# zhoujoey/ORB-SLAM3-Mac

Measured on AMD Instinct MI355X. Metric: ORB extract+match frames/sec, higher is better.
Workload: dtype u8; 1 GPU; vga: synthetic 640x480 batch=1024 per GPU, 8-level pyramid, 1000 feats/frame, ORB extract + Hamming 2-NN match (Frame.cc:1146) + SearchForInitialization (ORBmatcher.cc:710) vs successor frame; pipelines=1, matchers=side by side (two contexts), frames_total=1024

## Files before the change

include/orbhip.h:

```cpp
#ifndef ORBHIP_H
#define ORBHIP_H
#include <stddef.h>
#include <stdint.h>
#ifdef __cplusplus
extern "C" {
#endif

#define ORBHIP_OK 0
#define ORBHIP_E_BADARG (-1)
#define ORBHIP_E_NODEVICE (-2)
#define ORBHIP_E_HIP (-3)
#define ORBHIP_E_CAPACITY (-4)
#define ORBHIP_E_ABORTED (-5)
#define ORBHIP_E_NOTSPD (-6)
#define ORBHIP_E_EMPTY (-7)

typedef struct {
    float x, y, size, angle, response;
    int32_t octave, class_id;
} orbhip_keypoint;

typedef struct orbhip_ctx orbhip_ctx;
typedef struct orbhip_extractor orbhip_extractor;

// ... 3 lines not shown
int orbhip_ctx_create(int device, void *stream, orbhip_ctx **out);
void orbhip_ctx_destroy(orbhip_ctx *ctx);
int orbhip_ctx_synchronize(orbhip_ctx *ctx);
int orbhip_ctx_wait_for(orbhip_ctx *ctx, orbhip_ctx *other);
int orbhip_ctx_check_status(orbhip_ctx *ctx);
void *orbhip_ctx_stream(orbhip_ctx *ctx);

int orbhip_extractor_create(orbhip_ctx *ctx, int nfeatures, float scale_factor, int nlevels,
                            int ini_th_fast, int min_th_fast, orbhip_extractor **out);
void orbhip_extractor_destroy(orbhip_extractor *ext);

int orbhip_extractor_levels(const orbhip_extractor *ext);
int orbhip_extractor_table(const orbhip_extractor *ext, int which, float *out);
int orbhip_extractor_features_per_level(const orbhip_extractor *ext, int *out);
int orbhip_extractor_umax(const orbhip_extractor *ext, int *out16);

int orbhip_extractor_reserve(orbhip_extractor *ext, int width, int height, int max_batch);
int orbhip_extractor_max_keypoints(const orbhip_extractor *ext);

int orbhip_extract_batch_device(orbhip_extractor *ext, const uint8_t *d_images, int width,
                                int height, size_t row_stride, size_t frame_stride, int batch,
                                int lap0, int lap1);
int orbhip_extractor_results(orbhip_extractor *ext, orbhip_keypoint **d_kp, uint8_t **d_desc,
                             int32_t **d_count, int32_t **d_mono_index);
int orbhip_extract_batch_host(orbhip_extractor *ext, const uint8_t *h_images, int width, int height,
                              size_t row_stride, size_t frame_stride, int batch, int lap0, int lap1,
                              orbhip_keypoint *kp_out, uint8_t *desc_out, int cap,
                              int32_t *count_out, int32_t *mono_out);
int orbhip_extract_batch_host_view(orbhip_extractor *ext, const uint8_t *h_images, int width, int height, size_t row_stride,
                                   size_t frame_stride, int batch, int lap0, int lap1, const orbhip_keypoint **kp_view,
                                   const uint8_t **desc_view, int *row_capacity, const int32_t **count_view, const int32_t **mono_view);
int orbhip_extractor_blur_kernel(const orbhip_extractor *ext, int batch);

int orbhip_extractor_resize_band_rows(const orbhip_extractor *ext, int level);

int orbhip_extractor_last_frame(orbhip_extractor *ext, int frame, const orbhip_keypoint **d_kp, const uint8_t **d_desc,
                                const orbhip_keypoint **h_kp_view, const uint8_t **h_desc_view, int32_t *count, unsigned long long *generation);

int orbhip_extractor_level_dims(const orbhip_extractor *ext, int level, int *w, int *h);
int orbhip_extractor_get_pyramid_level(orbhip_extractor *ext, int frame, int level, int padded,
                                       uint8_t *h_out, size_t out_stride);
int orbhip_extractor_get_pyramid_padded(orbhip_extractor *ext, int frame, uint8_t *const *levels_out, const size_t *strides);
int orbhip_extractor_get_blurred_level(orbhip_extractor *ext, int frame, int level,
                                       uint8_t *h_out, size_t out_stride);
int orbhip_extractor_get_fast_candidates(orbhip_extractor *ext, int frame, int level,
                                         int32_t *xs, int32_t *ys, int32_t *scores, int cap,
                                         int32_t *n_out);
// ... 575 lines not shown
```

orb-slam3-mac_amd/csrc/orb_internal.h:

```cpp
#pragma once
#include <hip/hip_runtime.h>
#include <stdint.h>
#include "../../include/orbhip.h"

#define ORB_MAX_LEVELS 16
#define ORB_EDGE 19
#define ORB_MINB 16
#define ORB_HALF_PATCH 15
#define ORB_RS_STEPS 24

struct OrbLevel {
    uint8_t *img;
    uint8_t *blur;
    size_t img_frame_stride;
    size_t blur_frame_stride;
    int w, h, img_pitch, blur_pitch;
    int ncols, nrows, wcell, hcell;
    int cell_base;
    int cell_cap;
    int quota;
    int key_base, key_cap;
    int kp_base, kp_cap;
    int n_ini;
    float hx;
    float scale;
    float size;
    const int16_t *xofs; const int16_t *xalpha; const int16_t *yofs; const int16_t *ybeta;
    const uint32_t *xchunk; const uint32_t *ytab;
    int resize_mode;
    int rs_rows;
};
// ... 25 lines not shown
    float *lvl_angle;
    uint8_t *lvl_desc;
    int32_t *lvl_count;
    int32_t *lvl_ncand;
    int32_t *status;
    orbhip_keypoint *out_kp;
    uint8_t *out_desc;
    int32_t *out_count;
    int32_t *out_mono;
    int umax[ORB_HALF_PATCH + 1];
    int gauss_q8[7];
    const uint4 *bm_th;
    const uint4 *bm_tv;
    int bm_cols[ORB_MAX_LEVELS + 1];
    int bm_init;
};

struct FcLevel {
    const uint8_t *img; size_t frame_stride; int img_pitch;
    int max_bx, max_by;
    int ncols, nrows, wcell, hcell, cell_base, cell_cap;
    int tpr, rpt;
    int rpc, rpr, run_base;
};
struct FastParams {
    FcLevel lv[ORB_MAX_LEVELS];
    int nlevels, batch, ini_th, min_th, cells_per_frame;
    int n_cus;
    int chunk;
    int lvl_lo, lvl_hi;
    uint32_t *cell_count, *cell_list; size_t cell_list_frame_stride; int32_t *status;
    int rows, srows, qcap, wave_dw, small_cells;
    uint32_t div_magic[34];
    int runs_per_frame, run_rows, run_q0, run_dw, use_runs;
};

#define ORB_PACK_KEY(x, y, s) ((uint32_t)(x) | ((uint32_t)(y) << 12) | ((uint32_t)(s) << 24))
#define ORB_KEY_X(k) ((int)((k) & 0xFFFu))
#define ORB_KEY_Y(k) ((int)(((k) >> 12) & 0xFFFu))
#define ORB_KEY_S(k) ((int)((k) >> 24))

__device__ __forceinline__ int hamming256(const uint4 &a0, const uint4 &a1, const uint4 &b0, const uint4 &b1)
{
    return __popc(a0.x ^ b0.x) + __popc(a0.y ^ b0.y) + __popc(a0.z ^ b0.z) + __popc(a0.w ^ b0.w) +
           __popc(a1.x ^ b1.x) + __popc(a1.y ^ b1.y) + __popc(a1.z ^ b1.z) + __popc(a1.w ^ b1.w);
}

struct StereoLevel {
    const uint8_t *imgL, *imgR;
    size_t fsL, fsR;
    int pitchL, pitchR, wR, pad_;
// ... 33 lines not shown
```

orb-slam3-mac_amd/csrc/orb_kernels.hip:

```cpp
#include "orb_internal.h"
#include "wave_dpp.h"
#include <mutex>
#include <vector>
#include <cstdio>
#include <cstdlib>

#define WAVE 64

__device__ __forceinline__ int wave_incl_scan(int v) { return wave_scan_add_dpp(v); }

__device__ __forceinline__ int block_excl_scan256(int v, int *wsum, int *total)
{
    const int lane = threadIdx.x & (WAVE - 1), wid = threadIdx.x >> 6;
    int inc = wave_incl_scan(v);
    if (lane == WAVE - 1) wsum[wid] = inc;
    __syncthreads();
    int base = 0;
#pragma unroll
    for (int w = 0; w < 4; w++) {
        int s = wsum[w];
        if (w < wid) base += s;
    }
    *total = wsum[0] + wsum[1] + wsum[2] + wsum[3];
    __syncthreads();
// ... 1609 lines not shown
    const uint32_t khi = (uint32_t)P.gauss_q8[4] | ((uint32_t)P.gauss_q8[5] << 8) | ((uint32_t)P.gauss_q8[6] << 16);
    const uint32_t k0 = P.gauss_q8[0], k1 = P.gauss_q8[1], k2 = P.gauss_q8[2], k3 = P.gauss_q8[3];
    const uint32_t k01 = k0 | (k1 << 16), k23 = k2 | (k3 << 16), k21 = k2 | (k1 << 16);
    if (idx < nint * nb) {
        const int band = idx / nint, c = 1 + idx - band * nint;
        blr_band<false>(src, dst, L.img_pitch, L.blur_pitch, w, h, 4 * c, band * BLR_R, klo, khi, k01, k23, k21, k0);
    } else {
        const int e = idx - nint * nb, band = e / nedge, ce = e - band * nedge;
        const int c = ce == 0 ? 0 : nint + ce;
        blr_band<true>(src, dst, L.img_pitch, L.blur_pitch, w, h, 4 * c, band * BLR_R, klo, khi, k01, k23, k21, k0);
    }
}

typedef int v4i __attribute__((ext_vector_type(4)));
__device__ __forceinline__ v4i bm_as_v4i(uint4 v) { v4i r; r[0] = (int)v.x; r[1] = (int)v.y; r[2] = (int)v.z; r[3] = (int)v.w; return r; }
__global__ __launch_bounds__(256) void k_blur_mfma(OrbParams P, int frame0, int nframes)
{
    const int per_frame = P.bm_cols[P.nlevels];
    const unsigned wid = xcd_logical_id(blockIdx.x, gridDim.x) * 4 + (threadIdx.x >> 6);
    const int lane = threadIdx.x & 63, m = lane & 15, g = lane >> 4;
    const int fr = (int)(wid / (unsigned)per_frame), rem = (int)(wid - (unsigned)fr * (unsigned)per_frame);
    if (fr >= nframes) return;
    int level = 0;
    for (int l = 1; l < P.nlevels; l++) if (rem >= P.bm_cols[l]) level = l;
    const OrbLevel &L = P.lv[level];
    const int w = L.w, h = L.h, spitch = L.img_pitch, dpitch = L.blur_pitch;
    const int tx = rem - P.bm_cols[level], X0 = 32 * tx;
    const uint8_t *src = L.img + (size_t)(frame0 + fr) * L.img_frame_stride;
    uint8_t *dst = L.blur + (size_t)(frame0 + fr) * L.blur_frame_stride;
    int cx = X0 - 16 + 16 * g;
    cx = cx < 0 ? 0 : cx;
    if (cx + 16 > w) cx = w - 16;
    const uint4 *th = P.bm_th + ((size_t)(P.bm_cols[level] + tx) * 2) * 64 + lane;
    const v4i B0 = bm_as_v4i(th[0]), B1 = bm_as_v4i(th[64]);
    v4i TV[4];
#pragma unroll
    for (int b = 0; b < 4; b++) TV[b] = bm_as_v4i(P.bm_tv[b * 64 + lane]);
    const int init = P.bm_init;
    v4i c_init = {init, init, init, init}, c_init_lo = {init + 32768, init + 32768, init + 32768, init + 32768};
    asm volatile("" : "+v"(c_init), "+v"(c_init_lo));
    const int nty = (h + 57) / 58;
    auto load_window = [&](int Y0, u32x4_unaligned (&raw)[4]) {
// ... 30 lines not shown
                const uint32_t pab = __builtin_amdgcn_perm((uint32_t)C1[cb][t][1], (uint32_t)C1[cb][t][0], 0x05040100u);
                const uint32_t pcd = __builtin_amdgcn_perm((uint32_t)C1[cb][t][3], (uint32_t)C1[cb][t][2], 0x05040100u);
                Alo[t] = (int)(__builtin_amdgcn_perm(pcd, pab, 0x06040200u) ^ 0x80808080u);
                Ahi[t] = (int)(__builtin_amdgcn_perm(pcd, pab, 0x07050301u) ^ 0x80808080u);
            }
            const int col = X0 + 16 * cb + 4 * g;
#pragma unroll
            for (int b = 0; b < 4; b++) {
                const v4i Chi = __builtin_amdgcn_mfma_i32_16x16x64_i8(Ahi, TV[b], c_init, 0, 0, 0);
                const v4i Clo = __builtin_amdgcn_mfma_i32_16x16x64_i8(Alo, TV[b], c_init_lo, 0, 0, 0);
                uint32_t v[4];
#pragma unroll
                for (int r = 0; r < 4; r++) v[r] = min(((uint32_t)Chi[r] << 8) + (uint32_t)Clo[r], 0x00FFFFFFu);
                const uint32_t p01 = __builtin_amdgcn_perm(v[1], v[0], 0x0c0c0602u), p23 = __builtin_amdgcn_perm(v[3], v[2], 0x0c0c0602u);
                const int row = Y0 + 16 * b + m;
                if (16 * b + m < 58 && row < h && col < w) *reinterpret_cast<uint32_t *>(dst + (uint32_t)(__umul24((uint32_t)row, (uint32_t)dpitch) + (uint32_t)col)) = p01 | (p23 << 16);
            }
        }
    }
}

void orb_launch_blur(const OrbParams &P, hipStream_t s, int wgs_per_cu, int frame0, int nframes)
{
    if (P.bm_cols[P.nlevels] > 0 && P.batch >= P.bm_min_batch) {
        if (nframes < 0) nframes = P.batch - frame0;
        const long waves = (long)P.bm_cols[P.nlevels] * nframes;
        if (nframes > 0) hipLaunchKernelGGL(k_blur_mfma, dim3((unsigned)((waves + 3) / 4)), dim3(256), 0, s, P, frame0, nframes);
        return;
    }
    if (P.br_blocks[P.nlevels] > 0 && P.batch >= P.rows_min_batch) {
        if (nframes < 0) nframes = P.batch - frame0;
        if (nframes > 0) hipLaunchKernelGGL(k_blur_rows, dim3((unsigned)P.br_blocks[P.nlevels] * (unsigned)nframes), dim3(256), 0, s, P, frame0);
        return;
    }
    if (frame0 > 0) return;
    const long total = (long)P.bs_tiles[P.nlevels] * P.batch;
    long nblocks = (long)(P.n_cus > 0 ? P.n_cus : 256) * wgs_per_cu;
    if (nblocks > total) nblocks = total;
    hipLaunchKernelGGL(k_blur, dim3((unsigned)nblocks), dim3(256), 0, s, P);
}

__constant__ int8_t c_pattern[1024] = {
// ... 178 lines not shown
            const uint32_t c0 = __float_as_uint(__fadd_rn(__fsub_rn(__fmul_rn(pk.x, a), __fmul_rn(pk.y, b)), MAGIC));
            const uint32_t r1 = __float_as_uint(__fadd_rn(__fadd_rn(__fmul_rn(pk.z, b), __fmul_rn(pk.w, a)), MAGIC));
            const uint32_t c1 = __float_as_uint(__fadd_rn(__fsub_rn(__fmul_rn(pk.z, a), __fmul_rn(pk.w, b)), MAGIC));
            const uint32_t i0 = (r0 << 5) + (r0 << 4) + c0 + offk, i1 = (r1 << 5) + (r1 << 4) + c1 + offk;
            const uint32_t t0 = bp[i0], t1 = bp[i1];
            bits = __builtin_amdgcn_alignbit(bits, t0 - t1, 31);
        }
        if (valid) {
            uint8_t *desc = P.lvl_desc + ((size_t)frame * P.kps_per_frame + slot) * 32;
            reinterpret_cast<uint16_t *>(desc)[l16] = (uint16_t)bits;
            if (l16 == 0) P.lvl_angle[(size_t)frame * P.kps_per_frame + slot] = angle;
        }
    }
}

void orb_launch_orient_desc(const OrbParams &P, hipStream_t s)
{
    const long groups_x = (long)((P.batch + 7) / 8) * ((P.kps_per_frame + 3) >> 2);
    long blocks_x = (groups_x + (OD_THREADS / 64) - 1) / (OD_THREADS / 64);
    if (blocks_x > 4096) blocks_x = 4096;
    const long blocks = 8 * blocks_x;
    hipLaunchKernelGGL(k_orient_desc, dim3((unsigned)blocks), dim3(OD_THREADS), 0, s, P);
}

__global__ __launch_bounds__(256) void k_assemble(OrbParams P)
{
    __shared__ int wsum[8];
    __shared__ int s_cnt[ORB_MAX_LEVELS + 1];
    const int tid = threadIdx.x, frame = blockIdx.x;
    if (tid == 0) {
        int n = 0;
        for (int l = 0; l < P.nlevels; l++) { s_cnt[l] = n; n += P.lvl_count[frame * P.nlevels + l]; }
        s_cnt[P.nlevels] = n;
    }
    __syncthreads();
    const int n = s_cnt[P.nlevels];
    orbhip_keypoint *okp = P.out_kp + (size_t)frame * P.max_kp;
// ... 42 lines not shown
```

orb-slam3-mac_amd/csrc/orbhip_api.hip:

```cpp
#include "orb_internal.h"
#include "ctx_internal.h"
#include <cmath>
#include <cfloat>
#include <cstdio>
#include <cstdlib>
#include <cstring>
#include <string>
#include <vector>
#include <mutex>
#include <set>
#include <utility>

static thread_local std::string g_last_error;
extern "C" const char *orbhip_last_error(void) { return g_last_error.c_str(); }
extern "C" const char *orbhip_version(void) { return "orbhip 0.1 (gfx950)"; }

#define HIP_TRY(expr)                                                                   \
    do {                                                                                \
        hipError_t _e = (expr);                                                         \
        if (_e != hipSuccess) {                                                         \
            g_last_error = std::string(#expr) + ": " + hipGetErrorString(_e);           \
            return ORBHIP_E_HIP;                                                        \
        }                                                                               \
    } while (0)
// ... 334 lines not shown
    for (int d = 0; d < dn; d++) {
        float f = (float)((d + 0.5) * scale - 0.5);
        int s = (int)floorf(f);
        f -= s;
        if (horizontal) {
            if (s < 0) { f = 0; s = 0; }
            if (s >= sn - 1) { f = 0; s = sn - 1; }
        }
        int c0 = cv_round_f((1.f - f) * 2048), c1 = cv_round_f(f * 2048);
        ofs[d] = (int16_t)std::min(std::max(s, -32768), 32767);
        coef[2 * d] = (int16_t)std::min(std::max(c0, -32768), 32767);
        coef[2 * d + 1] = (int16_t)std::min(std::max(c1, -32768), 32767);
    }
}

extern "C" int orbhip_extractor_reserve(orbhip_extractor *e, int width, int height, int max_batch)
{
    if (!e || width <= 0 || height <= 0 || max_batch <= 0) return ORBHIP_E_BADARG;
    if (e->width == width && e->height == height && e->max_batch >= max_batch) return ORBHIP_OK;
    if (width > 4096 + 2 * ORB_MINB || height > 4096 + 2 * ORB_MINB) { g_last_error = "image larger than 12-bit key packing"; return ORBHIP_E_BADARG; }
    HIP_TRY(hipSetDevice(e->ctx->device));
    HIP_TRY(hipStreamSynchronize(e->ctx->stream));
    ext_free_all(e);
    OrbParams &P = e->P;
    memset(&P, 0, sizeof(P));
    P.nlevels = e->nlevels; P.ini_th = e->ini_th; P.min_th = e->min_th;
    memcpy(P.umax, e->umax, sizeof(P.umax));
    memcpy(P.gauss_q8, e->gauss_q8, sizeof(P.gauss_q8));
    int cells = 0, keys = 0, kps = 0, max_cell_cap = 0;
    for (int l = 0; l < e->nlevels; l++) {
// ... 75 lines not shown
        bool ok = !getenv("ORBHIP_BLUR_TILES");
        P.br_blocks[0] = 0;
        for (int l = 0; l < e->nlevels; l++) {
            const int w = P.lv[l].w, h = P.lv[l].h;
            if (h < BLR_R + 4 || w < 16) ok = false;
            P.br_blocks[l + 1] = P.br_blocks[l] + (((w + 3) / 4) * ((h + BLR_R - 1) / BLR_R) + 255) / 256;
        }
        if (!ok) P.br_blocks[e->nlevels] = 0;
    }
    P.cell_list_frame_stride = (size_t)cells * max_cell_cap;
    int rc;
    const size_t B = (size_t)max_batch;
    for (int l = 0; l < e->nlevels; l++) {
        OrbLevel &L = P.lv[l];
        L.img_pitch = align_up(L.w, 64); L.blur_pitch = L.img_pitch;
        L.img_frame_stride = (size_t)L.img_pitch * L.h; L.blur_frame_stride = L.img_frame_stride;
        if ((rc = dev_alloc(e, &L.img, B * L.img_frame_stride + 64))) return rc;
        if ((rc = dev_alloc(e, &L.blur, B * L.blur_frame_stride + 64))) return rc;
        if (l > 0) {
            std::vector<int16_t> xo, xa, yo, yb;
            resize_tables(P.lv[l - 1].w, L.w, true, xo, xa);
            resize_tables(P.lv[l - 1].h, L.h, false, yo, yb);
            int16_t *dxo, *dxa, *dyo, *dyb;
            if ((rc = dev_alloc(e, &dxo, xo.size()))) return rc;
            if ((rc = dev_alloc(e, &dxa, xa.size()))) return rc;
            if ((rc = dev_alloc(e, &dyo, yo.size()))) return rc;
            if ((rc = dev_alloc(e, &dyb, yb.size()))) return rc;
            HIP_TRY(hipMemcpy(dxo, xo.data(), xo.size() * 2, hipMemcpyHostToDevice));
            HIP_TRY(hipMemcpy(dxa, xa.data(), xa.size() * 2, hipMemcpyHostToDevice));
            HIP_TRY(hipMemcpy(dyo, yo.data(), yo.size() * 2, hipMemcpyHostToDevice));
            HIP_TRY(hipMemcpy(dyb, yb.data(), yb.size() * 2, hipMemcpyHostToDevice));
// ... 92 lines not shown
                            for (int g = 0; g < 4 && gp < 0; g++) if (col >= cxs[g] && col < cxs[g] + 16) gp = g;
                            if (gp < 0) { ok = false; break; }
                            int8_t &c = th[((((size_t)(P.bm_cols[l] + tx) * 2 + cb) * 64) + (size_t)(n + 16 * gp)) * 16 + (col - cxs[gp])];
                            c = (int8_t)(c + e->gauss_q8[i + 3]);
                        }
                    }
            }
        }
        for (int b = 0; b < 4; b++)
            for (int lane = 0; lane < 64; lane++)
                for (int j = 0; j < 16; j++) {
                    const int n = lane & 15, g = lane >> 4, krow = 16 * (j >> 2) + 4 * g + (j & 3), d = krow - (16 * b + n);
                    tv[((size_t)b * 64 + lane) * 16 + j] = (int8_t)((d >= 0 && d <= 6) ? e->gauss_q8[d] : 0);
                }
        P.bm_th = nullptr; P.bm_tv = nullptr; P.bm_init = 128 * S;
        if (ok) {
            uint4 *dth, *dtv;
            if ((rc = dev_alloc(e, &dth, th.size() / 16))) return rc;
            if ((rc = dev_alloc(e, &dtv, tv.size() / 16))) return rc;
            HIP_TRY(hipMemcpy(dth, th.data(), th.size(), hipMemcpyHostToDevice));
            HIP_TRY(hipMemcpy(dtv, tv.data(), tv.size(), hipMemcpyHostToDevice));
            P.bm_th = dth; P.bm_tv = dtv;
        } else P.bm_cols[e->nlevels] = 0;
    }
    if ((rc = dev_alloc(e, &P.cell_count, B * cells))) return rc;
    if ((rc = dev_alloc(e, &P.cell_list, B * P.cell_list_frame_stride))) return rc;
    if ((rc = dev_alloc(e, &P.keys, B * keys))) return rc;
    if ((rc = dev_alloc(e, &P.node_of, B * keys))) return rc;
    if ((rc = dev_alloc(e, &P.lvl_kp, B * kps))) return rc;
    if ((rc = dev_alloc(e, &P.lvl_perm, B * kps))) return rc;
    if ((rc = dev_alloc(e, &P.lvl_angle, B * kps))) return rc;
    if ((rc = dev_alloc(e, &P.lvl_desc, B * kps * 32))) return rc;
    if ((rc = dev_alloc(e, &P.lvl_count, B * e->nlevels))) return rc;
    if ((rc = dev_alloc(e, &P.lvl_ncand, B * e->nlevels))) return rc;
    if ((rc = dev_alloc(e, &P.status, 1))) return rc;
    {
        auto up = [](size_t v) { return (v + 255) & ~(size_t)255; };
        e->ob_kp = up(8 * B); e->ob_desc = e->ob_kp + up(sizeof(orbhip_keypoint) * B * P.max_kp);
        e->outblob_bytes = e->ob_desc + up((size_t)32 * B * P.max_kp);
// ... 151 lines not shown
    memcpy(depth_out, h + 2 * (size_t)max_n, 4 * (size_t)n_left);
    memcpy(x3d_out, h + 3 * (size_t)max_n, 12 * (size_t)n_left);
    if (n_matches_out) *n_matches_out = h[6 * (size_t)max_n];
    return ORBHIP_OK;
}

extern "C" int orbhip_extractor_blur_kernel(const orbhip_extractor *e, int batch)
{
    if (!e || !e->max_batch) return -1;
    const OrbParams &P = e->P;
    if (P.bm_cols[e->nlevels] > 0 && batch >= P.bm_min_batch) return 2;
    if (P.br_blocks[e->nlevels] > 0 && batch >= P.rows_min_batch) return 1;
    return 0;
}

extern "C" int orbhip_extractor_resize_band_rows(const orbhip_extractor *e, int level)
{
    if (!e || !e->max_batch || level < 1 || level >= e->nlevels) return -1;
    return e->P.lv[level].xchunk ? e->P.lv[level].rs_rows : 0;
}

extern "C" int orbhip_extractor_set_profiling(orbhip_extractor *e, int enable)
{
    if (!e) return ORBHIP_E_BADARG;
    if (enable && !e->ev_created) {
        for (auto &slot : e->ev) for (auto &ev : slot) HIP_TRY(hipEventCreate(&ev));
        e->ev_created = true;
    }
    e->profiling = enable != 0;
    e->ev_calls = 0;
// ... 12 lines not shown
            float ms = 0.f;
            HIP_TRY(hipEventElapsedTime(&ms, e->ev[slot][i], e->ev[slot][i + 1]));
            ms_out[i] += ms / n;
        }
    }
    e->ev_calls = 0;
    return ORBHIP_OK;
}

static int tune_int(const char *name, int dflt) { const char *v = getenv(name); return v ? atoi(v) : dflt; }

static int run_pipeline(orbhip_extractor *e, int batch, int lap0, int lap1)
{
    OrbParams &P = e->P;
    P.batch = batch; P.lap0 = lap0; P.lap1 = lap1; P.n_cus = e->ctx->n_cus;
    hipStream_t s = e->ctx->stream;
    const bool prof = e->profiling;
    const int slot = e->ev_calls % ORBHIP_PROF_SLOTS;
#define STAGE_MARK(i) do { if (prof) HIP_TRY(hipEventRecord(e->ev[slot][i], s)); } while (0)
    const bool fork = e->overlap && !prof && batch >= ORB_OVERLAP_MIN_BATCH;
    if (fork && !e->aux_ok) {
        HIP_TRY(hipStreamCreateWithFlags(&e->aux, hipStreamNonBlocking));
        HIP_TRY(hipEventCreateWithFlags(&e->ev_fork, hipEventDisableTiming));
        HIP_TRY(hipEventCreateWithFlags(&e->ev_join, hipEventDisableTiming));
        HIP_TRY(hipEventCreateWithFlags(&e->ev_pyr, hipEventDisableTiming));
        e->aux_ok = true;
    }
    FastParams &F = e->F;
    for (int l = 0; l < e->nlevels; l++) { F.lv[l].img = P.lv[l].img; F.lv[l].frame_stride = P.lv[l].img_frame_stride; F.lv[l].img_pitch = P.lv[l].img_pitch; }
    F.batch = batch; F.n_cus = e->ctx->n_cus; F.cell_count = P.cell_count; F.cell_list = P.cell_list; F.cell_list_frame_stride = P.cell_list_frame_stride; F.status = P.status;
// ... 280 lines not shown
        }
        for (int y = 0; y < ORB_EDGE; y++) {
            memcpy(base + (size_t)y * st, base + (size_t)(ORB_EDGE + reflect101_host(y - ORB_EDGE, L.h)) * st, (size_t)L.w + 2 * ORB_EDGE);
            memcpy(base + (size_t)(L.h + ORB_EDGE + y) * st, base + (size_t)(ORB_EDGE + reflect101_host(L.h + y, L.h)) * st, (size_t)L.w + 2 * ORB_EDGE);
        }
    }
    return ORBHIP_OK;
}

extern "C" int orbhip_extractor_get_blurred_level(orbhip_extractor *e, int frame, int level, uint8_t *h_out, size_t out_stride)
{
    if (!e || !h_out || level < 0 || level >= e->nlevels || frame < 0 || frame >= e->last_batch) return ORBHIP_E_BADARG;
    const OrbLevel &L = e->P.lv[level];
    HIP_TRY(hipSetDevice(e->ctx->device));
    HIP_TRY(hipStreamSynchronize(e->ctx->stream));
    HIP_TRY(hipMemcpy2D(h_out, out_stride, L.blur + (size_t)frame * L.blur_frame_stride, L.blur_pitch, L.w, L.h, hipMemcpyDeviceToHost));
    return ORBHIP_OK;
}

extern "C" int orbhip_extractor_get_fast_candidates(orbhip_extractor *e, int frame, int level, int32_t *xs, int32_t *ys,
                                                    int32_t *scores, int cap, int32_t *n_out)
{
    if (!e || level < 0 || level >= e->nlevels || frame < 0 || frame >= e->last_batch || !n_out) return ORBHIP_E_BADARG;
    const OrbParams &P = e->P;
    const OrbLevel &L = P.lv[level];
    HIP_TRY(hipSetDevice(e->ctx->device));
    HIP_TRY(hipStreamSynchronize(e->ctx->stream));
    int32_t n = 0;
    HIP_TRY(hipMemcpy(&n, P.lvl_ncand + frame * P.nlevels + level, sizeof(n), hipMemcpyDeviceToHost));
    *n_out = n;
// ... 86 lines not shown
```

orb-slam3-mac_amd/python/orbhip.py:

```python
import ctypes as C
import os
import numpy as np

try:
    import torch
except Exception:
    torch = None

_HERE = os.path.dirname(os.path.abspath(__file__))
LIB_DIR = os.path.join(os.path.dirname(_HERE), "lib")
LIB_PATH = os.path.join(LIB_DIR, "liborbhip.so")
SYNTH_PATH = os.path.join(LIB_DIR, "libsynth.so")

if not os.path.exists(LIB_PATH):
    raise ImportError(
        "liborbhip.so not built: run `python -c 'import __graft_entry__ as g; g.build()'` "
        "(there is no CPU fallback for the HIP path)")

lib = C.CDLL(LIB_PATH)

OK, E_BADARG, E_NODEVICE, E_HIP, E_CAPACITY, E_ABORTED, E_NOTSPD, E_EMPTY = 0, -1, -2, -3, -4, -5, -6, -7
STAGES = ["pyramid", "fast_cells", "blur", "octree", "desc", "assemble"]

KP_DTYPE = np.dtype([("x", "<f4"), ("y", "<f4"), ("size", "<f4"), ("angle", "<f4"),
# ... 2 lines not shown

vp, ci, cf, cd, sz = C.c_void_p, C.c_int, C.c_float, C.c_double, C.c_size_t
lib.orbhip_version.restype = C.c_char_p
lib.orbhip_last_error.restype = C.c_char_p
lib.orbhip_ctx_create.argtypes = [ci, vp, C.POINTER(vp)]
lib.orbhip_ctx_destroy.argtypes = [vp]
lib.orbhip_ctx_synchronize.argtypes = [vp]
lib.orbhip_ctx_stream.argtypes = [vp]
lib.orbhip_ctx_stream.restype = vp
lib.orbhip_extractor_create.argtypes = [vp, ci, cf, ci, ci, ci, C.POINTER(vp)]
lib.orbhip_extractor_destroy.argtypes = [vp]
lib.orbhip_extractor_levels.argtypes = [vp]
lib.orbhip_extractor_table.argtypes = [vp, ci, vp]
lib.orbhip_extractor_features_per_level.argtypes = [vp, vp]
lib.orbhip_extractor_umax.argtypes = [vp, vp]
lib.orbhip_extractor_reserve.argtypes = [vp, ci, ci, ci]
lib.orbhip_extractor_max_keypoints.argtypes = [vp]
lib.orbhip_extract_batch_device.argtypes = [vp, vp, ci, ci, sz, sz, ci, ci, ci]
lib.orbhip_extractor_results.argtypes = [vp, C.POINTER(vp), C.POINTER(vp), C.POINTER(vp), C.POINTER(vp)]
lib.orbhip_extract_batch_host.argtypes = [vp, vp, ci, ci, sz, sz, ci, ci, ci, vp, vp, ci, vp, vp]
lib.orbhip_extractor_level_dims.argtypes = [vp, ci, C.POINTER(ci), C.POINTER(ci)]
lib.orbhip_extractor_get_pyramid_level.argtypes = [vp, ci, ci, ci, vp, sz]
lib.orbhip_extractor_get_blurred_level.argtypes = [vp, ci, ci, vp, sz]
lib.orbhip_extractor_get_pyramid_padded.argtypes = [vp, ci, vp, vp]
lib.orbhip_extractor_get_fast_candidates.argtypes = [vp, ci, ci, vp, vp, vp, ci, C.POINTER(C.c_int32)]
lib.orbhip_extractor_get_level_keypoints.argtypes = [vp, ci, ci, vp, ci, C.POINTER(C.c_int32)]
lib.orbhip_extractor_set_profiling.argtypes = [vp, ci]
lib.orbhip_extractor_set_graph_mode.argtypes = [vp, ci]
lib.orbhip_extractor_stage_ms.argtypes = [vp, vp]
lib.orbhip_descriptor_distance.argtypes = [vp, vp]
lib.orbhip_match_bf2nn_device.argtypes = [vp, vp, vp, sz, vp, vp, sz, ci, ci, cd, vp, vp, vp]
lib.orbhip_search_for_initialization_device.argtypes = [vp, vp, vp, vp, vp, vp, vp, ci, ci, sz, cf, cf, cf, cf, ci, cf, ci,
                                                        vp, vp, vp]
lib.orbhip_ctx_check_status.argtypes = [vp]
lib.orbhip_ctx_wait_for.argtypes = [vp, vp]
lib.orbhip_extractor_blur_kernel.argtypes = [vp, ci]
lib.orbhip_extractor_blur_kernel.restype = ci
lib.orbhip_extractor_resize_band_rows.argtypes = [vp, ci]
lib.orbhip_extractor_resize_band_rows.restype = ci
if hasattr(lib, "orbhip_debug_octree"):
    lib.orbhip_debug_octree.argtypes = [vp, ci, ci, vp, vp, vp, vp, ci, vp, ci, vp, vp]
lib.orbhip_prev_matched_init_device.argtypes = [vp, vp, sz, ci, ci, vp]
lib.orbhip_search_by_projection_device.argtypes = [vp, vp, vp, vp, ci, vp, vp, vp, vp, ci, sz, ci, cf, cf, cf, cf, ci, ci, vp, vp]
lib.orbhip_search_local_map_device.argtypes = [vp, vp, vp, vp, ci, vp, vp, vp, vp, ci, sz, ci, cf, cf, cf, cf, ci, cf, vp, vp]


class OrbHipError(RuntimeError):
    def __init__(self, code, where):
        self.code = code
        super().__init__("%s failed: %d (%s)" % (where, code, lib.orbhip_last_error().decode()))


# ... 15 lines not shown
        _chk(lib.orbhip_ctx_check_status(self.h), "orbhip_ctx_check_status")

    def wait_for(self, other):
        _chk(lib.orbhip_ctx_wait_for(self.h, other.h), "orbhip_ctx_wait_for")

    @property
    def stream(self):
        return lib.orbhip_ctx_stream(self.h)

    def close(self):
        if self.h:
            lib.orbhip_ctx_destroy(self.h)
            self.h = None


class Extractor:

    def __init__(self, ctx, nfeatures=1000, scale_factor=1.2, nlevels=8, ini_th=20, min_th=7):
        h = vp()
        _chk(lib.orbhip_extractor_create(ctx.h, nfeatures, scale_factor, nlevels, ini_th, min_th, C.byref(h)),
             "orbhip_extractor_create")
        self.h, self.ctx, self.nlevels = h, ctx, nlevels

    def close(self):
        if self.h:
            lib.orbhip_extractor_destroy(self.h)
            self.h = None

    def table(self, which):
        out = np.zeros(self.nlevels, np.float32)
# ... 7 lines not shown

    def umax(self):
        out = np.zeros(16, np.int32)
        _chk(lib.orbhip_extractor_umax(self.h, out.ctypes.data), "umax")
        return out

    def reserve(self, w, h, batch):
        _chk(lib.orbhip_extractor_reserve(self.h, w, h, batch), "orbhip_extractor_reserve")

    @property
    def max_keypoints(self):
        return lib.orbhip_extractor_max_keypoints(self.h)

    def blur_kernel(self, batch):
        return ("k_blur", "k_blur_rows", "k_blur_mfma")[lib.orbhip_extractor_blur_kernel(self.h, int(batch))]

    def resize_band_rows(self, level):
        return lib.orbhip_extractor_resize_band_rows(self.h, int(level))

    def debug_octree(self, level, lists, form):
        offs = np.zeros(len(lists) + 1, np.int32)
        offs[1:] = np.cumsum([len(l[0]) for l in lists])
        xs, ys, ss = (np.ascontiguousarray(np.concatenate([np.asarray(l[k], np.int32) for l in lists] + [np.zeros(1, np.int32)])) for k in range(3))
        cap = int(max(len(l[0]) for l in lists)) + 16
        keys = np.zeros((len(lists), cap), np.uint32)
        counts, redo = np.zeros(len(lists), np.int32), np.zeros(len(lists), np.int32)
        _chk(lib.orbhip_debug_octree(self.h, int(level), len(lists), offs.ctypes.data, xs.ctypes.data, ys.ctypes.data, ss.ctypes.data,
                                     {"iterative": 0, "table": 1}[form], keys.ctypes.data, cap, counts.ctypes.data, redo.ctypes.data),
             "orbhip_debug_octree")
        kept = [np.stack([k & 0xFFF, (k >> 12) & 0xFFF, k >> 24], 1).astype(np.int32) for k in (keys[f, :counts[f]] for f in range(len(lists)))]
# ... 1114 lines not shown
```

Baseline: 339,300 frames/s.

## Store blurred pyramid in 16x8 tiles and read only pattern-covered rows

The MFMA blur kernel can now write the blurred image in a tiled layout of 16x8-byte tiles. A new orient/descriptor kernel reads the 37x37 blurred neighbourhood from those tiles as 16-byte loads, skipping chunks outside the circular reach of the BRIEF pattern through precomputed per-row half-widths. The goal is fewer wasted and scattered global loads in descriptor computation. In exchange it adds a second layout path, a larger blur buffer, and a host-side untiling step when reading blurred levels back for debugging.

```diff
diff --git a/include/orbhip.h b/include/orbhip.h
--- a/include/orbhip.h
+++ b/include/orbhip.h
@@ -41,6 +41,7 @@
 int orbhip_extractor_table(const orbhip_extractor *ext, int which, float *out);
 int orbhip_extractor_features_per_level(const orbhip_extractor *ext, int *out);
 int orbhip_extractor_umax(const orbhip_extractor *ext, int *out16);
+int orbhip_blur_half_widths(int *out19);
 
 int orbhip_extractor_reserve(orbhip_extractor *ext, int width, int height, int max_batch);
 int orbhip_extractor_max_keypoints(const orbhip_extractor *ext);
@@ -58,6 +59,7 @@
                                    size_t frame_stride, int batch, int lap0, int lap1, const orbhip_keypoint **kp_view,
                                    const uint8_t **desc_view, int *row_capacity, const int32_t **count_view, const int32_t **mono_view);
 int orbhip_extractor_blur_kernel(const orbhip_extractor *ext, int batch);
+int orbhip_extractor_blur_tiled(const orbhip_extractor *ext, int batch);
 
 int orbhip_extractor_resize_band_rows(const orbhip_extractor *ext, int level);
 
diff --git a/orb-slam3-mac_amd/csrc/orb_internal.h b/orb-slam3-mac_amd/csrc/orb_internal.h
--- a/orb-slam3-mac_amd/csrc/orb_internal.h
+++ b/orb-slam3-mac_amd/csrc/orb_internal.h
@@ -15,6 +15,7 @@
     size_t img_frame_stride;
     size_t blur_frame_stride;
     int w, h, img_pitch, blur_pitch;
+    int blur_tiles_x;
     int ncols, nrows, wcell, hcell;
     int cell_base;
     int cell_cap;
@@ -70,6 +71,9 @@
     const uint4 *bm_tv;
     int bm_cols[ORB_MAX_LEVELS + 1];
     int bm_init;
+    int blur_tiled_ok;
+    int blur_tiled;
+    int blur_hw[ORB_EDGE];
 };
 
 struct FcLevel {
@@ -91,6 +95,7 @@
     int runs_per_frame, run_rows, run_q0, run_dw, use_runs;
 };
 
+#define ORB_BLUR_TILE_OFF(x, y, tiles_x) ((((uint32_t)((y) >> 3) * (uint32_t)(tiles_x) + (uint32_t)((x) >> 4)) << 7) + (uint32_t)(((y) & 7) << 4) + (uint32_t)((x) & 15))
 #define ORB_PACK_KEY(x, y, s) ((uint32_t)(x) | ((uint32_t)(y) << 12) | ((uint32_t)(s) << 24))
 #define ORB_KEY_X(k) ((int)((k) & 0xFFFu))
 #define ORB_KEY_Y(k) ((int)(((k) >> 12) & 0xFFFu))
diff --git a/orb-slam3-mac_amd/csrc/orb_kernels.hip b/orb-slam3-mac_amd/csrc/orb_kernels.hip
--- a/orb-slam3-mac_amd/csrc/orb_kernels.hip
+++ b/orb-slam3-mac_amd/csrc/orb_kernels.hip
@@ -1647,6 +1647,7 @@
 
 typedef int v4i __attribute__((ext_vector_type(4)));
 __device__ __forceinline__ v4i bm_as_v4i(uint4 v) { v4i r; r[0] = (int)v.x; r[1] = (int)v.y; r[2] = (int)v.z; r[3] = (int)v.w; return r; }
+template <bool TILED>
 __global__ __launch_bounds__(256) void k_blur_mfma(OrbParams P, int frame0, int nframes)
 {
     const int per_frame = P.bm_cols[P.nlevels];
@@ -1658,7 +1659,7 @@
     for (int l = 1; l < P.nlevels; l++) if (rem >= P.bm_cols[l]) level = l;
     const OrbLevel &L = P.lv[level];
     const int w = L.w, h = L.h, spitch = L.img_pitch, dpitch = L.blur_pitch;
-    const int tx = rem - P.bm_cols[level], X0 = 32 * tx;
+    const int tx = rem - P.bm_cols[level], X0 = 32 * tx, tiles_x = L.blur_tiles_x;
     const uint8_t *src = L.img + (size_t)(frame0 + fr) * L.img_frame_stride;
     uint8_t *dst = L.blur + (size_t)(frame0 + fr) * L.blur_frame_stride;
     int cx = X0 - 16 + 16 * g;
@@ -1719,6 +1720,9 @@
                 for (int r = 0; r < 4; r++) v[r] = min(((uint32_t)Chi[r] << 8) + (uint32_t)Clo[r], 0x00FFFFFFu);
                 const uint32_t p01 = __builtin_amdgcn_perm(v[1], v[0], 0x0c0c0602u), p23 = __builtin_amdgcn_perm(v[3], v[2], 0x0c0c0602u);
                 const int row = Y0 + 16 * b + m;
+                if (TILED) {
+                    if (16 * b + m < 58 && row < h && col < w) *reinterpret_cast<uint32_t *>(dst + ORB_BLUR_TILE_OFF(col, row, tiles_x)) = p01 | (p23 << 16);
+                } else
                 if (16 * b + m < 58 && row < h && col < w) *reinterpret_cast<uint32_t *>(dst + (uint32_t)(__umul24((uint32_t)row, (uint32_t)dpitch) + (uint32_t)col)) = p01 | (p23 << 16);
             }
         }
@@ -1730,7 +1734,8 @@
     if (P.bm_cols[P.nlevels] > 0 && P.batch >= P.bm_min_batch) {
         if (nframes < 0) nframes = P.batch - frame0;
         const long waves = (long)P.bm_cols[P.nlevels] * nframes;
-        if (nframes > 0) hipLaunchKernelGGL(k_blur_mfma, dim3((unsigned)((waves + 3) / 4)), dim3(256), 0, s, P, frame0, nframes);
+        if (nframes > 0 && P.blur_tiled) hipLaunchKernelGGL(k_blur_mfma<true>, dim3((unsigned)((waves + 3) / 4)), dim3(256), 0, s, P, frame0, nframes);
+        else if (nframes > 0) hipLaunchKernelGGL(k_blur_mfma<false>, dim3((unsigned)((waves + 3) / 4)), dim3(256), 0, s, P, frame0, nframes);
         return;
     }
     if (P.br_blocks[P.nlevels] > 0 && P.batch >= P.rows_min_batch) {
@@ -1939,13 +1944,162 @@
     }
 }
 
+#define OD_TP 64
+#define OD_TROWS 40
+#define OD_KP_LDS_T ((OD_TROWS * OD_TP) / 4)
+__global__ __launch_bounds__(OD_THREADS) void k_orient_desc_tiled(OrbParams P)
+{
+    __shared__ __attribute__((aligned(16))) uint32_t lds_all[OD_THREADS / 16][OD_KP_LDS_T];
+    __shared__ float4 pat_t[16 * 16];
+    __shared__ int od_hw[48];
+    __shared__ uint32_t od_msk[16 * 8];
+    const int tid = threadIdx.x, lane = tid & 63, l16 = lane & 15, sub = lane >> 4;
+    for (int e = tid; e < 256; e += OD_THREADS) {
+        const int l = e & 15, t = e >> 4;
+        const int8_t *pp = &c_pattern[4 * (16 * l + t)];
+        pat_t[t * 16 + l] = make_float4((float)pp[0], (float)pp[1], (float)pp[2], (float)pp[3]);
+    }
+    if (tid < 16 * 8) {
+        const int d = P.umax[tid >> 3], j = tid & 7;
+        uint32_t m = 0;
+        for (int k = 0; k < 4; k++) { const int u = -ORB_HALF_PATCH + 4 * j + k; if (u >= -d && u <= d) m |= 0xFFu << (8 * k); }
+        od_msk[tid] = m;
+    }
+    if (tid < 48) { const int r = tid - 3, d = r < 18 ? 18 - r : r - 18; od_hw[tid] = (r >= 0 && r <= 36) ? P.blur_hw[d] : -64; }
+    int uhw[6];
+#pragma unroll
+    for (int k = 0; k < 6; k++) { const int i = l16 + 16 * k, r = (i * 43) >> 7, d = r < 15 ? 15 - r : r - 15; uhw[k] = i < 31 * 3 ? P.umax[d] : -64; }
+    __syncthreads();
+    const int xcd = blockIdx.x & 7, nblk_x = gridDim.x >> 3;
+    const long wave_x = (long)(blockIdx.x >> 3) * (OD_THREADS / 64) + (tid >> 6), nwaves_x = (long)nblk_x * (OD_THREADS / 64);
+    const int gpf = (P.kps_per_frame + 3) >> 2;
+    const int nframes_x = (P.batch - xcd + 7) >> 3;
+    uint32_t *up32 = lds_all[(tid >> 4)], *bp32 = up32;
+    const uint8_t *bp = reinterpret_cast<const uint8_t *>(bp32);
+    const float factor_pi = (float)(3.1415926535897932384626433832795 / 180.f);
+    const long ngroups = (long)nframes_x * gpf;
+    for (long q = wave_x; q < ngroups; q += nwaves_x) {
+        const int fk = __builtin_amdgcn_readfirstlane((int)(q / gpf));
+        const int frame = xcd + 8 * fk;
+        const int slot0 = __builtin_amdgcn_readfirstlane(4 * (int)(q - (long)fk * gpf));
+        int lvl = 0;
+        for (int l = 1; l < P.nlevels; l++) if (slot0 >= P.lv[l].kp_base) lvl = l;
+        lvl = __builtin_amdgcn_readfirstlane(lvl);
+        const OrbLevel &L = P.lv[lvl];
+        const int slot_w = slot0 + sub;
+        const int nk = P.lvl_count[frame * P.nlevels + lvl];
+        const bool valid = (slot_w - L.kp_base) < nk;
+        const int slot = (valid && P.batch >= ORB_PERM_MIN_BATCH) ? L.kp_base + (int)P.lvl_perm[(size_t)frame * P.kps_per_frame + slot_w] : slot_w;
+        if (slot0 - L.kp_base >= nk) continue;
+        int x = 19, y = 19;
+        if (valid) {
+            const uint32_t key = P.lvl_kp[(size_t)frame * P.kps_per_frame + slot];
+            x = ORB_KEY_X(key) + ORB_MINB; y = ORB_KEY_Y(key) + ORB_MINB;
+        }
+        const int uxs = (x - 15) & ~3, uoff = (x - 15) - uxs;
+        const int tc0 = (x - 18) >> 4, boff = (x - 18) & 15, yoff = (y - 18) & 3;
+        __builtin_amdgcn_fence(__ATOMIC_RELEASE, "wavefront");
+        uint4 br[10];
+        uint32_t bmask = 0, umask = 0;
+#pragma unroll
+        for (int k = 0; k < 10; k++) br[k] = make_uint4(0, 0, 0, 0);
+        int bhw[10];
+#pragma unroll
+        for (int k = 0; k < 10; k++) bhw[k] = od_hw[4 * k + (l16 & 3) - yoff + 3];
+        if (valid) {
+            const uint8_t *uimg = L.img + (size_t)frame * L.img_frame_stride, *bimg = L.blur + (size_t)frame * L.blur_frame_stride;
+            const int upitch = L.img_pitch & 0xFFFF, tiles_x = L.blur_tiles_x & 0xFFFF;
+            const uint32_t urow = (uint32_t)(((y - 15) & 0xFFFF) * upitch);
+            const int blo = 16 * (l16 >> 2) - 18 - boff;
+            uint4 ur[6];
+#pragma unroll
+            for (int k = 0; k < 6; k++) {
+                const int i = l16 + 16 * k, r = (i * 43) >> 7, c3 = i - r * 3;
+                const int ulo = 16 * c3 - 15 - uoff;
+                const bool on = ulo <= uhw[k] && ulo + 15 >= -uhw[k];
+                ur[k] = on ? od_load16(uimg, urow + (uint32_t)(r * upitch), uxs + 16 * c3) : make_uint4(0, 0, 0, 0);
+                umask |= on ? 1u << k : 0u;
+            }
+#pragma unroll
+            for (int k = 0; k < 10; k++) {
+                const int gy = y - 18 - yoff + (l16 & 3) + 4 * k;
+                if (blo <= bhw[k] && blo + 15 >= -bhw[k]) {
+                    br[k] = *reinterpret_cast<const uint4 *>(bimg + ((((uint32_t)(gy >> 3) * (uint32_t)tiles_x + (uint32_t)(tc0 + (l16 >> 2))) << 7) + (uint32_t)((gy & 7) << 4)));
+                    bmask |= 1u << k;
+                }
+            }
+#pragma unroll
+            for (int k = 0; k < 6; k++) {
+                const int i = l16 + 16 * k, r = (i * 43) >> 7, c3 = i - r * 3;
+                if (umask & (1u << k)) *reinterpret_cast<uint4 *>(&up32[r * (OD_UP / 4) + 4 * c3]) = ur[k];
+            }
+        }
+        __builtin_amdgcn_fence(__ATOMIC_RELEASE, "wavefront");
+        __builtin_amdgcn_s_waitcnt(0xc07f);
+        __builtin_amdgcn_wave_barrier();
+        __builtin_amdgcn_fence(__ATOMIC_ACQUIRE, "wavefront");
+        int m10, m01 = 0;
+        {
+            const int j = l16 & 7, par = l16 >> 3;
+            const uint32_t wts = 0x04030201u + 0x04040404u * (uint32_t)j;
+            uint32_t accP = 0, accS = 0;
+#pragma unroll 4
+            for (int i = 0; i < 16; i++) {
+                const int v = -ORB_HALF_PATCH + 2 * i + par, vc = min(v, ORB_HALF_PATCH);
+                const uint32_t *rq = up32 + (vc + ORB_HALF_PATCH) * (OD_UP / 4) + j;
+                uint32_t wv = __builtin_amdgcn_alignbyte(rq[1], rq[0], (uint32_t)uoff) & od_msk[(vc < 0 ? -vc : vc) * 8 + j];
+                if (v > ORB_HALF_PATCH) wv = 0;
+                const uint32_t sr = __builtin_amdgcn_udot4(wv, 0x01010101u, 0u, false);
+                accP = __builtin_amdgcn_udot4(wv, wts, accP, false);
+                accS += sr;
+                m01 += v * (int)sr;
+            }
+            m10 = (int)accP - 16 * (int)accS;
+        }
+        __builtin_amdgcn_fence(__ATOMIC_RELEASE, "wavefront");
+        __builtin_amdgcn_wave_barrier();
+#pragma unroll
+        for (int k = 0; k < 10; k++)
+            if (bmask & (1u << k)) *reinterpret_cast<uint4 *>(&bp32[((l16 & 3) + 4 * k) * (OD_TP / 4) + 4 * (l16 >> 2)]) = br[k];
+        m10 = row16_allreduce_add_dpp(m10); m01 = row16_allreduce_add_dpp(m01);
+        const float angle = fast_atan2_deg((float)m01, (float)m10);
+        double sd, cd;
+        sincos_det((double)__fmul_rn(angle, factor_pi), &sd, &cd);
+        const float a = (float)cd, b = (float)sd;
+        __builtin_amdgcn_fence(__ATOMIC_RELEASE, "wavefront");
+        __builtin_amdgcn_s_waitcnt(0xc07f);
+        __builtin_amdgcn_wave_barrier();
+        __builtin_amdgcn_fence(__ATOMIC_ACQUIRE, "wavefront");
+        const float MAGIC = 12582912.0f;
+        const uint32_t offk = (uint32_t)((18 + yoff) * OD_TP + boff + 18) - 65u * 0x4B400000u;
+        uint32_t bits = 0;
+#pragma unroll 4
+        for (int t = 15; t >= 0; t--) {
+            const float4 pk = pat_t[t * 16 + l16];
+            const uint32_t r0 = __float_as_uint(__fadd_rn(__fadd_rn(__fmul_rn(pk.x, b), __fmul_rn(pk.y, a)), MAGIC));
+            const uint32_t c0 = __float_as_uint(__fadd_rn(__fsub_rn(__fmul_rn(pk.x, a), __fmul_rn(pk.y, b)), MAGIC));
+            const uint32_t r1 = __float_as_uint(__fadd_rn(__fadd_rn(__fmul_rn(pk.z, b), __fmul_rn(pk.w, a)), MAGIC));
+            const uint32_t c1 = __float_as_uint(__fadd_rn(__fsub_rn(__fmul_rn(pk.z, a), __fmul_rn(pk.w, b)), MAGIC));
+            const uint32_t i0 = (r0 << 6) + c0 + offk, i1 = (r1 << 6) + c1 + offk;
+            const uint32_t t0 = bp[i0], t1 = bp[i1];
+            bits = __builtin_amdgcn_alignbit(bits, t0 - t1, 31);
+        }
+        if (valid) {
+            uint8_t *desc = P.lvl_desc + ((size_t)frame * P.kps_per_frame + slot) * 32;
+            reinterpret_cast<uint16_t *>(desc)[l16] = (uint16_t)bits;
+            if (l16 == 0) P.lvl_angle[(size_t)frame * P.kps_per_frame + slot] = angle;
+        }
+    }
+}
+
 void orb_launch_orient_desc(const OrbParams &P, hipStream_t s)
 {
     const long groups_x = (long)((P.batch + 7) / 8) * ((P.kps_per_frame + 3) >> 2);
     long blocks_x = (groups_x + (OD_THREADS / 64) - 1) / (OD_THREADS / 64);
     if (blocks_x > 4096) blocks_x = 4096;
     const long blocks = 8 * blocks_x;
-    hipLaunchKernelGGL(k_orient_desc, dim3((unsigned)blocks), dim3(OD_THREADS), 0, s, P);
+    if (P.blur_tiled) hipLaunchKernelGGL(k_orient_desc_tiled, dim3((unsigned)blocks), dim3(OD_THREADS), 0, s, P);
+    else hipLaunchKernelGGL(k_orient_desc, dim3((unsigned)blocks), dim3(OD_THREADS), 0, s, P);
 }
 
 __global__ __launch_bounds__(256) void k_assemble(OrbParams P)
diff --git a/orb-slam3-mac_amd/csrc/orbhip_api.hip b/orb-slam3-mac_amd/csrc/orbhip_api.hip
--- a/orb-slam3-mac_amd/csrc/orbhip_api.hip
+++ b/orb-slam3-mac_amd/csrc/orbhip_api.hip
@@ -372,6 +372,21 @@
     }
 }
 
+extern "C" int orbhip_blur_half_widths(int *out19)
+{
+    if (!out19) return ORBHIP_E_BADARG;
+    static const int8_t pat[1024] = {
+#include "orb_pattern.inc"
+    };
+    double R2 = 0;
+    for (int i = 0; i < 512; i++) R2 = std::max(R2, (double)pat[2 * i] * pat[2 * i] + (double)pat[2 * i + 1] * pat[2 * i + 1]);
+    for (int d = 0; d < ORB_EDGE; d++) {
+        const double t = std::max(d - 0.5, 0.0), q = R2 - t * t;
+        out19[d] = q > 0 ? std::min((int)floor(sqrt(q) + 0.5), 18) : -64;
+    }
+    return ORBHIP_OK;
+}
+
 extern "C" int orbhip_extractor_reserve(orbhip_extractor *e, int width, int height, int max_batch)
 {
     if (!e || width <= 0 || height <= 0 || max_batch <= 0) return ORBHIP_E_BADARG;
@@ -477,7 +492,9 @@
     for (int l = 0; l < e->nlevels; l++) {
         OrbLevel &L = P.lv[l];
         L.img_pitch = align_up(L.w, 64); L.blur_pitch = L.img_pitch;
-        L.img_frame_stride = (size_t)L.img_pitch * L.h; L.blur_frame_stride = L.img_frame_stride;
+        L.img_frame_stride = (size_t)L.img_pitch * L.h;
+        L.blur_tiles_x = (L.w + 15) / 16;
+        L.blur_frame_stride = align_up(std::max((size_t)L.blur_pitch * L.h, (size_t)L.blur_tiles_x * ((L.h + 7) / 8) * 128), (size_t)128);
         if ((rc = dev_alloc(e, &L.img, B * L.img_frame_stride + 64))) return rc;
         if ((rc = dev_alloc(e, &L.blur, B * L.blur_frame_stride + 64))) return rc;
         if (l > 0) {
@@ -600,6 +617,7 @@
                     tv[((size_t)b * 64 + lane) * 16 + j] = (int8_t)((d >= 0 && d <= 6) ? e->gauss_q8[d] : 0);
                 }
         P.bm_th = nullptr; P.bm_tv = nullptr; P.bm_init = 128 * S;
+        P.blur_tiled_ok = !(getenv("ORBHIP_BLUR_TILED") && atoi(getenv("ORBHIP_BLUR_TILED")) == 0);
         if (ok) {
             uint4 *dth, *dtv;
             if ((rc = dev_alloc(e, &dth, th.size() / 16))) return rc;
@@ -609,6 +627,7 @@
             P.bm_th = dth; P.bm_tv = dtv;
         } else P.bm_cols[e->nlevels] = 0;
     }
+    orbhip_blur_half_widths(P.blur_hw);
     if ((rc = dev_alloc(e, &P.cell_count, B * cells))) return rc;
     if ((rc = dev_alloc(e, &P.cell_list, B * P.cell_list_frame_stride))) return rc;
     if ((rc = dev_alloc(e, &P.keys, B * keys))) return rc;
@@ -790,6 +809,13 @@
     return 0;
 }
 
+extern "C" int orbhip_extractor_blur_tiled(const orbhip_extractor *e, int batch)
+{
+    if (!e || !e->max_batch) return -1;
+    const OrbParams &P = e->P;
+    return P.blur_tiled_ok && P.bm_cols[e->nlevels] > 0 && batch >= P.bm_min_batch ? 1 : 0;
+}
+
 extern "C" int orbhip_extractor_resize_band_rows(const orbhip_extractor *e, int level)
 {
     if (!e || !e->max_batch || level < 1 || level >= e->nlevels) return -1;
@@ -832,6 +858,7 @@
 {
     OrbParams &P = e->P;
     P.batch = batch; P.lap0 = lap0; P.lap1 = lap1; P.n_cus = e->ctx->n_cus;
+    P.blur_tiled = orbhip_extractor_blur_tiled(e, batch) == 1;
     hipStream_t s = e->ctx->stream;
     const bool prof = e->profiling;
     const int slot = e->ev_calls % ORBHIP_PROF_SLOTS;
@@ -1142,6 +1169,15 @@
     const OrbLevel &L = e->P.lv[level];
     HIP_TRY(hipSetDevice(e->ctx->device));
     HIP_TRY(hipStreamSynchronize(e->ctx->stream));
+    if (orbhip_extractor_blur_tiled(e, e->last_batch) == 1) {
+        const int tiles_x = L.blur_tiles_x, tiles_y = (L.h + 7) / 8;
+        std::vector<uint8_t> t((size_t)tiles_x * tiles_y * 128);
+        HIP_TRY(hipMemcpy(t.data(), L.blur + (size_t)frame * L.blur_frame_stride, t.size(), hipMemcpyDeviceToHost));
+        for (int y = 0; y < L.h; y++)
+            for (int x = 0; x < L.w; x += 16)
+                memcpy(h_out + (size_t)y * out_stride + x, t.data() + ORB_BLUR_TILE_OFF(x, y, tiles_x), (size_t)std::min(16, L.w - x));
+        return ORBHIP_OK;
+    }
     HIP_TRY(hipMemcpy2D(h_out, out_stride, L.blur + (size_t)frame * L.blur_frame_stride, L.blur_pitch, L.w, L.h, hipMemcpyDeviceToHost));
     return ORBHIP_OK;
 }
diff --git a/orb-slam3-mac_amd/python/orbhip.py b/orb-slam3-mac_amd/python/orbhip.py
--- a/orb-slam3-mac_amd/python/orbhip.py
+++ b/orb-slam3-mac_amd/python/orbhip.py
@@ -40,6 +40,7 @@
 lib.orbhip_extractor_table.argtypes = [vp, ci, vp]
 lib.orbhip_extractor_features_per_level.argtypes = [vp, vp]
 lib.orbhip_extractor_umax.argtypes = [vp, vp]
+lib.orbhip_blur_half_widths.argtypes = [vp]
 lib.orbhip_extractor_reserve.argtypes = [vp, ci, ci, ci]
 lib.orbhip_extractor_max_keypoints.argtypes = [vp]
 lib.orbhip_extract_batch_device.argtypes = [vp, vp, ci, ci, sz, sz, ci, ci, ci]
@@ -62,6 +63,8 @@
 lib.orbhip_ctx_wait_for.argtypes = [vp, vp]
 lib.orbhip_extractor_blur_kernel.argtypes = [vp, ci]
 lib.orbhip_extractor_blur_kernel.restype = ci
+lib.orbhip_extractor_blur_tiled.argtypes = [vp, ci]
+lib.orbhip_extractor_blur_tiled.restype = ci
 lib.orbhip_extractor_resize_band_rows.argtypes = [vp, ci]
 lib.orbhip_extractor_resize_band_rows.restype = ci
 if hasattr(lib, "orbhip_debug_octree"):
@@ -107,6 +110,12 @@
             self.h = None
 
 
+def blur_half_widths():
+    out = np.zeros(19, np.int32)
+    _chk(lib.orbhip_blur_half_widths(out.ctypes.data), "orbhip_blur_half_widths")
+    return out
+
+
 class Extractor:
 
     def __init__(self, ctx, nfeatures=1000, scale_factor=1.2, nlevels=8, ini_th=20, min_th=7):
@@ -144,6 +153,9 @@
 
     def blur_kernel(self, batch):
         return ("k_blur", "k_blur_rows", "k_blur_mfma")[lib.orbhip_extractor_blur_kernel(self.h, int(batch))]
+
+    def blur_tiled(self, batch):
+        return lib.orbhip_extractor_blur_tiled(self.h, int(batch)) == 1
 
     def resize_band_rows(self, level):
         return lib.orbhip_extractor_resize_band_rows(self.h, int(level))
```

Measured after the change: 346,900 frames/s (median of 6 runs). +2.2%, better.
